# balcilar/gnn-matlang

Hardware: AMD Instinct MI355X
Metric: GNNML3 training graphs/sec on ZINC-12k (higher is better)
Workload: dtype f32 storage/accumulate; forward products fp32-class (edge branch bf16x6, conv f16x3 split), backward products bf16x3 split; 1 GPU; Zinc12k.py GNNML3 regression train step (4x ML3Layer 30+2, S=8 supports, learnedge, add-pool, L1-sum, Adam 1e-3), ZINC-like synthetic graphs; graphs_per_gpu=131072, global_batch=131072, nodes_per_gpu=3005312, support_edges_per_gpu=18320896, supports=8, parallelism=dp1, params=33309

## Files before the change

### gnn_matlang_amd/csrc/gml_spectconv_bwd3_impl.h

```cpp
#pragma once
#include <type_traits>
#include "gml_common.h"
#include "gml_spectconv_bwd_impl.h"

__host__ __device__ __forceinline__ int gml_wkey3(int o) { return ((o >> 3) & 1) << 1; }
__host__ __device__ __forceinline__ int gml_tkey3(int pos) { return ((pos >> 2) & 1) | ((((pos >> 1) ^ (pos >> 2) ^ (pos >> 3)) & 1) << 1); }

template <int S, int NFB, int NW, int NOB = 2>
struct GmlBwd3Cfg {
    static constexpr int ROWS = 16 * NW, NT = 64 * NW;
    static constexpr int ECAP_MAX = (S > 8 ? 12 : (S == 6 ? 16 : 8)) * ROWS;
    static constexpr int XCAP_MAX = 224;
    static constexpr int LDG = 16 * NOB + 4;
    static constexpr int NIMG = NFB > 2 ? 2 : 1;
    static constexpr int W_IMG = S * 16 * NOB * 32;
    static constexpr int W_HALF = NIMG * W_IMG;
    static constexpr int W_BYTES = 2 * W_HALF * 2;
    static constexpr int SS = (S % 4 == 0) ? 4 : ((S % 3 == 0) ? 3 : S);
    static constexpr int NSLAB = S / SS;
    static constexpr int NBLK = SS * NFB * NOB;
    static constexpr int BPW = (NBLK + NW - 1) / NW;
    static constexpr int XT_IMG = 2 * ROWS * 64;
    static constexpr int XT_BYTES = NIMG * XT_IMG;
    static constexpr int PT_BYTES = 2 * SS * ROWS * 64;
    static constexpr int GREC = 4 + ROWS / 4;
    static constexpr bool ASHARE = NW % (NOB * NFB) == 0;
    static constexpr bool OK = (S % SS == 0) && (NFB >= 1 && NFB <= 3) && NW == 8 && (NOB == 1 || NOB == 2) &&
                               (NFB < 3 || (NOB == 2 && S <= 6));
    __host__ __device__ static size_t stage_bytes(int ecap, int xcap) { return (size_t)ecap * S * 4 + (size_t)xcap * LDG * 4; }
    __host__ __device__ static size_t r_bytes(int ecap, int xcap) {
        const size_t a = stage_bytes(ecap, xcap);
        return a > (size_t)PT_BYTES ? a : (size_t)PT_BYTES;
    }
    static constexpr bool VALG = NOB == 2 && NW == 8 && (S == 8 || ((S == 6 || S == 4) && NFB == 3));
    __host__ __device__ static size_t lds_bytes(int ecap, int xcap) {
        if (VALG) return (size_t)W_BYTES + (ROWS + 8) * 4 + (size_t)ecap * 4 + (size_t)xcap * LDG * 4 + XT_BYTES + PT_BYTES;
        return (size_t)W_BYTES + (ROWS + 8) * 4 + (size_t)ecap * 4 + r_bytes(ecap, xcap) + XT_BYTES;
    }
};

#ifndef GML_ABL
#define GML_ABL 0
#endif

#ifdef GML_BWD2_TIMING
#define GML_T3(i) do { const unsigned t_ = (unsigned)__builtin_readcyclecounter(); tacc_[i] += t_ - tprev_; tprev_ = t_; } while (0)
#else
#define GML_T3(i)
#endif

#define GML_DPP9_(ctrl)                                                                                                          \
    asm("s_nop 1\n\tv_add_f32_dpp %0, %0, %0 " ctrl " row_mask:0xf bank_mask:0xf\n\tv_add_f32_dpp %1, %1, %1 " ctrl " row_mask:0xf bank_mask:0xf\n\t" \
        "v_add_f32_dpp %2, %2, %2 " ctrl " row_mask:0xf bank_mask:0xf\n\tv_add_f32_dpp %3, %3, %3 " ctrl " row_mask:0xf bank_mask:0xf\n\t"           \
        "v_add_f32_dpp %4, %4, %4 " ctrl " row_mask:0xf bank_mask:0xf\n\tv_add_f32_dpp %5, %5, %5 " ctrl " row_mask:0xf bank_mask:0xf\n\t"           \
        "v_add_f32_dpp %6, %6, %6 " ctrl " row_mask:0xf bank_mask:0xf\n\tv_add_f32_dpp %7, %7, %7 " ctrl " row_mask:0xf bank_mask:0xf\n\t"           \
        "v_add_f32_dpp %8, %8, %8 " ctrl " row_mask:0xf bank_mask:0xf"                                                         \
        : "+v"(v[0]), "+v"(v[1]), "+v"(v[2]), "+v"(v[3]), "+v"(v[4]), "+v"(v[5]), "+v"(v[6]), "+v"(v[7]), "+v"(v[8]))
__device__ __forceinline__ void gml_row16_sum9(float (&v)[9]) {
    GML_DPP9_("quad_perm:[1,0,3,2]");
    GML_DPP9_("quad_perm:[2,3,0,1]");
    GML_DPP9_("row_half_mirror");
    GML_DPP9_("row_mirror");
}

#ifndef GML_HADV
#define GML_HADV 0
#endif
#define GML_BWD3_HAD_LDS(ROWS_, NW_) (16 + (ROWS_) * 16 + (NW_) * 36 * 4)

template <int S, int NFB, int NW, bool XV, bool DZ = false, int NOB = 2, bool HAD = false>
__global__ __launch_bounds__(64 * NW, 2) void gml_k_spectconv_bwd3(const GmlBwdParams p) {
    static_assert(!HAD || (XV && NOB == 2 && NFB == 2 && S >= 2), "the fused output stage is compiled for the ZINC shape class");
    using C = GmlBwd3Cfg<S, NFB, NW, NOB>;
    constexpr int NH = 2 * NOB, GC = 4 * NOB;
    static_assert(!DZ || NOB == 2, "the dz hand-over is compiled for the ZINC shape class");
    constexpr int LDG = C::LDG, ROWS = C::ROWS, NT = C::NT, SS = C::SS, BPW = C::BPW;
    constexpr int VAL_ALIGN = (S % 4 == 0) ? 4 : ((S % 2 == 0) ? 2 : 1);
    constexpr bool VALG = C::VALG;
    constexpr bool DIRECT = NOB == 2 && (S == 8 || VALG);
    constexpr bool LATEC = VALG && C::NSLAB == 2;
    constexpr bool BUFLD = S == 8 && NOB == 2 && XV;
    extern __shared__ __attribute__((aligned(16))) unsigned char lds_raw[];
    __bf16* W_h = reinterpret_cast<__bf16*>(lds_raw);
    __bf16* W_l = W_h + C::W_HALF;
    int* rp_l = reinterpret_cast<int*>(lds_raw + C::W_BYTES);
    int* col_l = rp_l + ROWS + 8;
    unsigned char* rreg = reinterpret_cast<unsigned char*>(col_l + p.ecap);
    float* ea_l = reinterpret_cast<float*>(rreg);
    float* gs = VALG ? ea_l : ea_l + (size_t)p.ecap * S;
    unsigned char* xT = VALG ? rreg + (size_t)p.xcap * LDG * 4 : rreg + C::r_bytes(p.ecap, p.xcap);
    unsigned char* pT = VALG ? xT + C::XT_BYTES : rreg;
    float* wm_l = reinterpret_cast<float*>(VALG ? pT + C::PT_BYTES : xT + C::XT_BYTES);
    float* hb_l = wm_l + 128;
    float* dzf = hb_l + 4;
    float* bsum = dzf + ROWS * 4;

    const int tid = threadIdx.x;
    const int lane = tid & 63, wave = tid >> 6;
    const int r16 = lane & 15, kq = lane >> 4;
    const int wg = gml_xcd_remap(blockIdx.x, gridDim.x);
    const int g0 = wg * p.groups_per_wg;
    const int g1 = min(g0 + p.groups_per_wg, p.ngroups);

    if constexpr (DZ || HAD) {
        if (tid < 128) wm_l[tid] = ((tid >> 5) < p.nmix && (tid & 31) < p.Fin) ? ((tid >> 5) < p.nmix1 ? p.wmix[(tid >> 5) * p.Fin + (tid & 31)] : p.wmix2[((tid >> 5) - p.nmix1) * p.Fin + (tid & 31)]) : 0.f;
    }
    if constexpr (HAD) {
        if (tid < 4) hb_l[tid] = tid < 2 ? (p.hb11 ? p.hb11[tid] : 0.f) : (p.hb12 ? p.hb12[tid - 2] : 0.f);
        if (tid < NW * 36) bsum[tid] = 0.f;
    }
    constexpr int WO = 16 * NOB;
    constexpr int NIMG = C::NIMG;
    for (int e = tid; e < NIMG * S * WO * 32; e += NT) {
        const int fl = e & 31, o = (e >> 5) % WO, s = ((e >> 5) / WO) % S, img = (e >> 5) / (WO * S);
        const int f = 32 * img + fl;
        const float v = (f < p.Fin && o < p.Fout) ? p.w[((int64_t)s * p.Fin + f) * p.Fout + o] : 0.f;
        const __bf16 h = (__bf16)v;
        const __bf16 l = (__bf16)(v - (float)h);
        const int i = img * C::W_IMG + (s * WO + o) * 32 + ((((fl >> 3) ^ gml_wkey3(o)) & 3) << 3) + (fl & 7);
        W_h[i] = h; W_l[i] = l;
    }

    f32x4 dwacc[C::NSLAB][BPW];
#pragma unroll
    for (int i = 0; i < C::NSLAB; ++i)
#pragma unroll
        for (int j = 0; j < BPW; ++j) dwacc[i][j] = f32x4{0.f, 0.f, 0.f, 0.f};

#ifdef GML_BWD2_TIMING
    unsigned tacc_[12] = {0, 0, 0, 0, 0, 0, 0, 0, 0, 0, 0, 0};
    unsigned tprev_ = (unsigned)__builtin_readcyclecounter();
#endif
    constexpr int VW = (S % 4 == 0) ? 4 : ((S % 2 == 0) ? 2 : 1);
    typedef typename std::conditional<VW == 4, f32x4, f32x2>::type EV;
    constexpr int NC = C::ECAP_MAX / NT, NE4 = (VW > 1) ? C::ECAP_MAX * (S / VW) / NT : 1;
    constexpr int NG4 = (C::XCAP_MAX * GC + NT - 1) / NT;
    const int etot = p.rowptr[p.nrows];
    const int* colb = etot > 0 ? p.col : p.ginfo;
    const EV* valb = etot > 0 ? reinterpret_cast<const EV*>(p.val) : reinterpret_cast<const EV*>(p.ginfo);
    const int emax = max(etot, 1) - 1;
    const int64_t emax4 = (VW > 1) ? max((int64_t)etot * (S / VW), (int64_t)1) - 1 : 0;
    const int o4max = p.gvec ? ((p.Fout + 3) / 4 * 4 - 4) : 0;
    int cv[NC], rpv = 0, row_n = 0;
    EV ev4[NE4];
    f32x4 gv4[NG4];
    float xb[8];
    float xb2[NIMG == 2 ? 8 : 1];
    float gown[HAD ? 8 : 1];
    auto vec_group = [&](const int4 gi) {
        return (VW > 1) && p.gvec && gi.y <= C::ECAP_MAX && gi.w <= C::XCAP_MAX;
    };
    int4 gi_nv = int4{0, 0, 0, 0};
    int4 gi_c = int4{0, 0, 0, 0};
    auto latch = [&]() {
        gi_c = int4{__builtin_amdgcn_readfirstlane(gi_nv.x), __builtin_amdgcn_readfirstlane(gi_nv.y),
                    __builtin_amdgcn_readfirstlane(gi_nv.z), __builtin_amdgcn_readfirstlane(gi_nv.w)};
    };
    const int voff_g = (tid / GC) * (int)p.ldg * 4 + (tid % GC) * 16;
    auto issue = [&](int g) {
        const int64_t r0 = (int64_t)g * ROWS;
        const int4 gi = gi_c;
        const int kb = gi.x, ne = gi.y, lo = gi.z, nwin = gi.w;
        if constexpr (BUFLD) {
            auto rsrc = [](const void* base, int64_t nbytes) {
                return __builtin_amdgcn_make_buffer_rsrc(const_cast<void*>(base), 0, (int)(nbytes < 0 ? 0 : (nbytes > 0x7fffff00 ? 0x7fffff00 : nbytes)), 0x00020000);
            };
            const int64_t rem = (int64_t)etot - kb;
            const auto rs_rp = rsrc(p.rowptr + r0, (p.nrows + 1 - r0) * 4);
            const auto rs_col = rsrc(p.col + kb, rem * 4);
            const auto rs_val = rsrc(p.val + (int64_t)kb * S, rem * (S * 4));
            const auto rs_g = rsrc(p.g + (int64_t)lo * p.ldg, (p.nrows - lo) * p.ldg * 4);
            const auto rs_x = rsrc(p.x + r0 * p.ldx, (p.nrows - r0) * p.ldx * 4);
            const int ldxb = (int)p.ldx * 4, ldgb = (int)p.ldg * 4;
#pragma unroll
            for (int q4 = 0; q4 < 2; ++q4) {
                const u32x4 t = __builtin_amdgcn_raw_buffer_load_b128(rs_x, row_n * ldxb + 32 * kq + 16 * q4, 0, 0);
                xb[4 * q4] = __uint_as_float(t.x); xb[4 * q4 + 1] = __uint_as_float(t.y);
                xb[4 * q4 + 2] = __uint_as_float(t.z); xb[4 * q4 + 3] = __uint_as_float(t.w);
            }
            if constexpr (HAD && !(GML_HADV & 2)) {
                const auto rs_go = rsrc(p.g + r0 * p.ldg, (p.nrows - r0) * p.ldg * 4);
#pragma unroll
                for (int q4 = 0; q4 < 2; ++q4) {
                    const u32x4 t = __builtin_amdgcn_raw_buffer_load_b128(rs_go, row_n * ldgb + 32 * kq + 16 * q4, 0, 0);
                    gown[4 * q4] = __uint_as_float(t.x); gown[4 * q4 + 1] = __uint_as_float(t.y);
                    gown[4 * q4 + 2] = __uint_as_float(t.z); gown[4 * q4 + 3] = __uint_as_float(t.w);
                }
            }
            rpv = (int)__builtin_amdgcn_raw_buffer_load_b32(rs_rp, tid * 4, 0, 0);
#pragma unroll
            for (int t = 0; t < NC; ++t) cv[t] = (int)__builtin_amdgcn_raw_buffer_load_b32(rs_col, tid * 4, NT * 4 * t, 0);
#pragma unroll
            for (int t = 0; t < (VALG ? 0 : NE4); ++t) ev4[t] = __builtin_bit_cast(EV, __builtin_amdgcn_raw_buffer_load_b128(rs_val, tid * 16, NT * 16 * t, 0));
#pragma unroll
            for (int t = 0; t < NG4; ++t) gv4[t] = __builtin_bit_cast(f32x4, __builtin_amdgcn_raw_buffer_load_b128(rs_g, voff_g, t * (NT / GC) * ldgb, 0));
            return;
        }
        if constexpr (XV) {
            const float* xr = p.x + min(r0 + row_n, p.nrows - 1) * p.ldx;
            const int f4max = (p.Fin + 3) / 4 * 4 - 4;
#pragma unroll
            for (int q4 = 0; q4 < 2; ++q4) {
                const f32x4 t = *reinterpret_cast<const f32x4*>(xr + min(8 * kq + 4 * q4, f4max));
                xb[4 * q4] = t.x; xb[4 * q4 + 1] = t.y; xb[4 * q4 + 2] = t.z; xb[4 * q4 + 3] = t.w;
                if constexpr (NIMG == 2) {
                    const f32x4 u = *reinterpret_cast<const f32x4*>(xr + min(32 + 8 * kq + 4 * q4, f4max));
                    xb2[4 * q4] = u.x; xb2[4 * q4 + 1] = u.y; xb2[4 * q4 + 2] = u.z; xb2[4 * q4 + 3] = u.w;
                }
            }
        }
        if constexpr (HAD && !(GML_HADV & 2)) {
            const float* gr = p.g + min(r0 + row_n, p.nrows - 1) * p.ldg + 8 * kq;
#pragma unroll
            for (int q4 = 0; q4 < 2; ++q4) {
                const f32x4 t = *reinterpret_cast<const f32x4*>(gr + 4 * q4);
                gown[4 * q4] = t.x; gown[4 * q4 + 1] = t.y; gown[4 * q4 + 2] = t.z; gown[4 * q4 + 3] = t.w;
            }
        }
        rpv = p.rowptr[min(r0 + tid, p.nrows)];
        const int ne1 = max(ne, 1) - 1, ne41 = max(ne * (S / (VW > 1 ? VW : 1)), 1) - 1, nw1 = max(nwin, 1) - 1;
#pragma unroll
        for (int t = 0; t < NC; ++t) cv[t] = colb[min(kb + min(tid + NT * t, ne1), emax)];
#pragma unroll
        for (int t = 0; t < (VALG ? 0 : NE4); ++t) ev4[t] = valb[min((int64_t)kb * (S / (VW > 1 ? VW : 1)) + min(tid + NT * t, ne41), emax4)];
#pragma unroll
        for (int t = 0; t < NG4; ++t) {
            const int i = tid + NT * t;
            const int64_t rr = min((int64_t)lo + min(i / GC, nw1), p.nrows - 1);
            gv4[t] = *reinterpret_cast<const f32x4*>(p.g + rr * p.ldg + min((i % GC) * 4, o4max));
        }
    };
    auto load_rows = [&](int g) {
        const int32_t* rec = p.ginfo + (int64_t)g * C::GREC;
        gi_nv = *reinterpret_cast<const int4*>(rec);
        row_n = reinterpret_cast<const unsigned char*>(rec + 4)[wave * 16 + r16];
    };
    auto commit = [&](const int4 gi, const int nr) {
        const int kb = gi.x, ne = gi.y, lo = gi.z, nwin = gi.w;
        if (tid <= nr) rp_l[tid] = rpv;
        if (vec_group(gi)) {
#pragma unroll
            for (int t = 0; t < NC; ++t) { const int i = tid + NT * t; if (i < ne) col_l[i] = cv[t] - lo; }
#pragma unroll
            for (int t = 0; t < (VALG ? 0 : NE4); ++t) {
                const int i = tid + NT * t;
                if (i < ne * (S / (VW > 1 ? VW : 1))) reinterpret_cast<EV*>(ea_l)[i] = ev4[t];
            }
#pragma unroll
            for (int t = 0; t < NG4; ++t) {
                const int i = tid + NT * t;
                if (i < nwin * GC)
                    *reinterpret_cast<f32x4*>(gs + (i / GC) * LDG + (i % GC) * 4) = ((i % GC) * 4 < p.Fout) ? gv4[t] : f32x4{0.f, 0.f, 0.f, 0.f};
            }
        } else {
            for (int i = tid; i < ne; i += NT) col_l[i] = p.col[kb + i] - lo;
            if constexpr (!VALG)
                for (int i = tid; i < ne * S; i += NT) ea_l[i] = p.val[(int64_t)kb * S + i];
            for (int i = tid; i < nwin * 16 * NOB; i += NT) {
                const int rr = i / (16 * NOB), o = i % (16 * NOB);
                gs[rr * LDG + o] = (o < p.Fout) ? p.g[(int64_t)(lo + rr) * p.ldg + o] : 0.f;
            }
        }
    };
    if (g0 < g1) { load_rows(g0); latch(); issue(g0); }
    if constexpr (LATEC) {
        if (g0 < g1) commit(gi_c, (int)min((int64_t)ROWS, p.nrows - (int64_t)g0 * ROWS));
        __syncthreads();
    }
    if constexpr (HAD && !LATEC) __syncthreads();
    for (int g = g0; g < g1; ++g) {
        const int64_t r0 = (int64_t)g * ROWS;
        const int nr = (int)min((int64_t)ROWS, p.nrows - r0);
        const int4 gi = gi_c;
        const int kb = gi.x, ne = gi.y, lo = gi.z, nwin = gi.w;
        const int row = row_n;
        load_rows((GML_ABL & 1) ? g0 : min(g + 1, g1 - 1));
        const auto vrs = __builtin_amdgcn_make_buffer_rsrc(const_cast<float*>(VALG ? p.val + (int64_t)kb * S : p.x), 0, VALG ? ne * (S * 4) : 0, 0x00020000);
        uint32_t vtouch = 0;
        if constexpr (VALG) vtouch = __builtin_amdgcn_raw_buffer_load_b32(vrs, tid * 128, 0, 0);
        if constexpr (!VALG) __syncthreads();
        GML_T3(0);

        const bool rvalid = row < nr;
        if constexpr (!XV) {
            const float* xr = p.x + (r0 + row) * p.ldx + 8 * kq;
#pragma unroll
            for (int t = 0; t < 8; ++t) xb[t] = (rvalid && 8 * kq + t < p.Fin) ? xr[t] : 0.f;
            if constexpr (NIMG == 2) {
#pragma unroll
                for (int t = 0; t < 8; ++t) xb2[t] = (rvalid && 32 + 8 * kq + t < p.Fin) ? xr[32 + t] : 0.f;
            }
        }
        f32x4 dzv = f32x4{0.f, 0.f, 0.f, 0.f};
        float had_a[4], had_g6 = 0.f, had_g7 = 0.f, had_bs[9];
        const int pos_h = wave * 16 + r16;
        auto had_pre = [&]() {
#pragma unroll
            for (int j = 0; j < 8; ++j) {
                if (!(rvalid && 8 * kq + j < p.Fin)) xb[j] = 0.f;
                if ((!BUFLD && !rvalid) || (GML_HADV & 2)) gown[j] = 0.f;
            }
#pragma unroll
            for (int q = 0; q < 4; ++q) {
                const f32x4 w0 = *reinterpret_cast<const f32x4*>(wm_l + q * 32 + 8 * kq);
                const f32x4 w1 = *reinterpret_cast<const f32x4*>(wm_l + q * 32 + 8 * kq + 4);
                f32x2 a2 = f32x2{xb[0], xb[1]} * f32x2{w0.x, w0.y};
                a2 = f32x2{xb[2], xb[3]} * f32x2{w0.z, w0.w} + a2;
                a2 = f32x2{xb[4], xb[5]} * f32x2{w1.x, w1.y} + a2;
                a2 = f32x2{xb[6], xb[7]} * f32x2{w1.z, w1.w} + a2;
                had_a[q] = a2.x + a2.y;
            }
            had_g6 = __shfl(gown[6], r16 + 48); had_g7 = __shfl(gown[7], r16 + 48);
        };
        auto had_valu = [&]() {
            const auto a01 = __builtin_amdgcn_permlane16_swap(__float_as_uint(had_a[0]), __float_as_uint(had_a[1]), false, false);
            const auto a23 = __builtin_amdgcn_permlane16_swap(__float_as_uint(had_a[2]), __float_as_uint(had_a[3]), false, false);
            const float c01 = __uint_as_float(a01[0]) + __uint_as_float(a01[1]);
            const float c23 = __uint_as_float(a23[0]) + __uint_as_float(a23[1]);
            const auto bq = __builtin_amdgcn_permlane32_swap(__float_as_uint(c01), __float_as_uint(c23), false, false);
            const float pre = __uint_as_float(bq[0]) + __uint_as_float(bq[1]) + hb_l[kq];
            float th, dh;
            gml_tanh_d(pre, th, dh);
            const auto tsw = __builtin_amdgcn_permlane32_swap(__float_as_uint(th), __float_as_uint(th), false, false);
            const float tpart = __uint_as_float(kq < 2 ? tsw[1] : tsw[0]);
            const float dzo = (GML_HADV & 4) ? 0.f : ((kq & 1) ? had_g7 : had_g6) * tpart * dh;
            dzf[pos_h * 4 + kq] = dzo;
            if constexpr (!(GML_HADV & 1)) {
#pragma unroll
                for (int j = 0; j < 8; ++j) had_bs[j] = gown[j];
                had_bs[8] = dzo;
                gml_row16_sum9(had_bs);
            }
        };
        auto had_post = [&]() {
            if constexpr (!(GML_HADV & 1)) {
                if (r16 == 0) {
                    float* bw = bsum + wave * 36;
                    f32x4 o0 = *reinterpret_cast<const f32x4*>(bw + 8 * kq), o1 = *reinterpret_cast<const f32x4*>(bw + 8 * kq + 4);
                    o0 += f32x4{had_bs[0], had_bs[1], had_bs[2], had_bs[3]};
                    o1 += f32x4{had_bs[4], had_bs[5], had_bs[6], had_bs[7]};
                    *reinterpret_cast<f32x4*>(bw + 8 * kq) = o0;
                    *reinterpret_cast<f32x4*>(bw + 8 * kq + 4) = o1;
                    bw[32 + kq] += had_bs[8];
                }
            }
            dzv = *reinterpret_cast<const f32x4*>(dzf + pos_h * 4);
        };
        if constexpr (!LATEC) commit(gi, nr);
        bf16x8 xh, xl;
        bf16x8 xh2, xl2;
        unsigned xpos = 0;
        f32x2 Z[S][NH], P[S][NH];
        auto zproj = [&]() {
        if constexpr (HAD) had_pre();
        if constexpr (XV) {
#pragma unroll
            for (int j = 0; j < 8; ++j)
                if (!(rvalid && 8 * kq + j < p.Fin)) xb[j] = 0.f;
        }
        gml_split8(xb, xh, xl);
        if constexpr (NIMG == 2) {
#pragma unroll
            for (int j = 0; j < 8; ++j)
                if (!(rvalid && 32 + 8 * kq + j < p.Fin)) xb2[j] = 0.f;
            gml_split8(xb2, xh2, xl2);
        }
        if constexpr (DZ) {
#pragma unroll
            for (int j = 0; j < 8; ++j) xpos |= (xb[j] > 0.f ? 1u : 0u) << j;
        }

        {
            const int oa0 = NOB == 2 ? 8 * (r16 >> 2) + (r16 & 3) : r16;
            bf16x8 wh[2][NOB], wl[2][NOB];
            bf16x8 wh2[2][NIMG == 2 ? NOB : 1], wl2[2][NIMG == 2 ? NOB : 1];
            auto frag = [&](int s, int st) {
#pragma unroll
                for (int ob = 0; ob < NOB; ++ob) {
                    const int oa = oa0 + 4 * ob;
                    const int off = (s * WO + oa) * 32 + (((kq ^ gml_wkey3(oa)) & 3) << 3);
                    wh[st][ob] = *reinterpret_cast<const bf16x8*>(W_h + off);
                    wl[st][ob] = *reinterpret_cast<const bf16x8*>(W_l + off);
                    if constexpr (NIMG == 2) {
                        wh2[st][ob] = *reinterpret_cast<const bf16x8*>(W_h + C::W_IMG + off);
                        wl2[st][ob] = *reinterpret_cast<const bf16x8*>(W_l + C::W_IMG + off);
                    }
                }
            };
            if (!(GML_ABL & 16)) frag(0, 0);
            if constexpr (HAD) had_valu();
#pragma unroll
            for (int s = 0; s < S; ++s) {
                const int st = s & 1;
                if (GML_ABL & 16) {
#pragma unroll
                    for (int h = 0; h < NH; ++h) { Z[s][h] = f32x2{xb[h], xb[h + 4]}; P[s][h] = f32x2{0.f, 0.f}; }
                    continue;
                }
                if (s + 1 < S) frag(s + 1, st ^ 1);
                f32x4 dd[NOB];
#pragma unroll
                for (int ob = 0; ob < NOB; ++ob) dd[ob] = f32x4{0.f, 0.f, 0.f, 0.f};
#pragma unroll
                for (int ob = 0; ob < NOB; ++ob) dd[ob] = __builtin_amdgcn_mfma_f32_16x16x32_bf16(wl[st][ob], xh, dd[ob], 0, 0, 0);
#pragma unroll
                for (int ob = 0; ob < NOB; ++ob) dd[ob] = __builtin_amdgcn_mfma_f32_16x16x32_bf16(wh[st][ob], xl, dd[ob], 0, 0, 0);
#pragma unroll
                for (int ob = 0; ob < NOB; ++ob) dd[ob] = __builtin_amdgcn_mfma_f32_16x16x32_bf16(wh[st][ob], xh, dd[ob], 0, 0, 0);
                if constexpr (NIMG == 2) {
#pragma unroll
                    for (int ob = 0; ob < NOB; ++ob) dd[ob] = __builtin_amdgcn_mfma_f32_16x16x32_bf16(wl2[st][ob], xh2, dd[ob], 0, 0, 0);
#pragma unroll
                    for (int ob = 0; ob < NOB; ++ob) dd[ob] = __builtin_amdgcn_mfma_f32_16x16x32_bf16(wh2[st][ob], xl2, dd[ob], 0, 0, 0);
#pragma unroll
                    for (int ob = 0; ob < NOB; ++ob) dd[ob] = __builtin_amdgcn_mfma_f32_16x16x32_bf16(wh2[st][ob], xh2, dd[ob], 0, 0, 0);
                }
#pragma unroll
                for (int ob = 0; ob < NOB; ++ob) { Z[s][2 * ob] = f32x2{dd[ob][0], dd[ob][1]}; Z[s][2 * ob + 1] = f32x2{dd[ob][2], dd[ob][3]}; }
#pragma unroll
                for (int h = 0; h < NH; ++h) asm volatile("v_pk_mov_b32 %0, 0, 0" : "=v"(P[s][h]));
            }
            __builtin_amdgcn_sched_group_barrier(0x100, 2 * NOB * NIMG, 0);
#pragma unroll
            for (int s = 0; s < S; ++s) {
                if (s + 1 < S) __builtin_amdgcn_sched_group_barrier(0x100, 2 * NOB * NIMG, 0);
                __builtin_amdgcn_sched_group_barrier(0x008, 3 * NOB * NIMG, 0);
            }
        }
        if constexpr (HAD) had_post();
        };
        if constexpr (!LATEC) __syncthreads();
        GML_T3(1);
        f32x4 dxa[NFB];
        const bool dxv = p.dx && p.dxvec;
        if constexpr (DZ) {
            if constexpr (!HAD) dzv = *reinterpret_cast<const f32x4*>(p.dz + min(r0 + row, p.nrows - 1) * 4);
        } else if constexpr (!HAD) {
            const float* dxb = p.dx ? p.dx : p.x;
            const int64_t ldb = p.dx ? p.lddx : p.ldx;
            const float* dr = dxb + min(r0 + row, p.nrows - 1) * ldb;
            if (dxv) {
                const int f4max = (p.Fin + 3) / 4 * 4 - 4;
#pragma unroll
                for (int fb = 0; fb < NFB; ++fb) dxa[fb] = *reinterpret_cast<const f32x4*>(dr + min(16 * fb + 4 * kq, f4max));
            } else {
#pragma unroll
                for (int fb = 0; fb < NFB; ++fb)
#pragma unroll
                    for (int reg = 0; reg < 4; ++reg) dxa[fb][reg] = dr[min(16 * fb + 4 * kq + reg, p.Fin - 1)];
            }
        }

        const int kbeg = rvalid ? rp_l[row] - kb : 0;
        const int kend = rvalid ? rp_l[row + 1] - kb : 0;

        zproj();
        GML_T3(2);
        const auto dvrs = __builtin_amdgcn_make_buffer_rsrc(const_cast<float*>(DIRECT && p.dval ? p.dval + (int64_t)kb * S : p.x), 0,
                                                            (DIRECT && p.dval && !(GML_ABL & 8)) ? ne * (S * 4) : 0, 0x00020000);
        auto ldg_row = [&](int dstl, f32x2 (&gv)[NH]) {
#pragma unroll
            for (int ob = 0; ob < NOB; ++ob) {
                const f32x4 t0 = *reinterpret_cast<const f32x4*>(gs + dstl * LDG + 4 * NOB * kq + 4 * ob);
                gv[2 * ob] = f32x2{t0.x, t0.y}; gv[2 * ob + 1] = f32x2{t0.z, t0.w};
            }
        };
        auto edge_g = [&](int k, const float (&ev)[S], const f32x2 (&gv)[NH]) {
            float d[S];
#pragma unroll
            for (int s = 0; s < S; ++s) {
                f32x2 a2 = f32x2{0.f, 0.f};
                const f32x2 e2 = f32x2{ev[s], ev[s]};
#pragma unroll
                for (int h = 0; h < NH; ++h) {
                    P[s][h] = e2 * gv[h] + P[s][h];
                    a2 = Z[s][h] * gv[h] + a2;
                }
                d[s] = a2.x + a2.y;
            }
            if constexpr (DIRECT && S == 4) {
                const auto a01 = __builtin_amdgcn_permlane16_swap(__float_as_uint(d[0]), __float_as_uint(d[1]), false, false);
                const auto a23 = __builtin_amdgcn_permlane16_swap(__float_as_uint(d[2]), __float_as_uint(d[3]), false, false);
                const float c01 = __uint_as_float(a01[0]) + __uint_as_float(a01[1]);
                const float c23 = __uint_as_float(a23[0]) + __uint_as_float(a23[1]);
                const auto b = __builtin_amdgcn_permlane32_swap(__float_as_uint(c01), __float_as_uint(c23), false, false);
                __builtin_amdgcn_raw_buffer_store_b32(__float_as_uint(__uint_as_float(b[0]) + __uint_as_float(b[1])), dvrs, (k * S + kq) * 4, 0, 0);
            } else if constexpr (DIRECT) {
                float tot2[2];
#pragma unroll
                for (int c = 0; c < 2; ++c) {
                    const float d6 = (S > 6) ? d[(S > 6) ? 6 + c : 0] : 0.f;
                    const auto a01 = __builtin_amdgcn_permlane16_swap(__float_as_uint(d[c]), __float_as_uint(d[2 + c]), false, false);
                    const auto a23 = __builtin_amdgcn_permlane16_swap(__float_as_uint(d[4 + c]), __float_as_uint(d6), false, false);
                    const float c01 = __uint_as_float(a01[0]) + __uint_as_float(a01[1]);
                    const float c23 = __uint_as_float(a23[0]) + __uint_as_float(a23[1]);
                    const auto b = __builtin_amdgcn_permlane32_swap(__float_as_uint(c01), __float_as_uint(c23), false, false);
                    tot2[c] = __uint_as_float(b[0]) + __uint_as_float(b[1]);
                }
                typedef uint32_t u32x2_ __attribute__((ext_vector_type(2)));
                const int doff = (S == 8 || kq < S / 2) ? (k * S + 2 * kq) * 4 : 0x7ffffff0;
                __builtin_amdgcn_raw_buffer_store_b64(u32x2_{__float_as_uint(tot2[0]), __float_as_uint(tot2[1])}, dvrs, doff, 0, 0);
            } else {
#pragma unroll
            for (int c = 0; c < (S + 3) / 4; ++c) {
                const float v0 = d[4 * c], v1 = (4 * c + 1 < S) ? d[4 * c + 1] : 0.f;
                const float v2 = (4 * c + 2 < S) ? d[4 * c + 2] : 0.f, v3 = (4 * c + 3 < S) ? d[4 * c + 3] : 0.f;
                const auto a01 = __builtin_amdgcn_permlane16_swap(__float_as_uint(v0), __float_as_uint(v1), false, false);
                const auto a23 = __builtin_amdgcn_permlane16_swap(__float_as_uint(v2), __float_as_uint(v3), false, false);
                const float c01 = __uint_as_float(a01[0]) + __uint_as_float(a01[1]);
                const float c23 = __uint_as_float(a23[0]) + __uint_as_float(a23[1]);
                const auto b = __builtin_amdgcn_permlane32_swap(__float_as_uint(c01), __float_as_uint(c23), false, false);
                const float tot = __uint_as_float(b[0]) + __uint_as_float(b[1]);
                if (4 * c + kq < S) ea_l[k * S + 4 * c + kq] = tot;
            }
            }
        };
        auto edge = [&](int k, const float (&ev)[S]) {
            f32x2 gv[NH];
            ldg_row(col_l[k], gv);
            edge_g(k, ev, gv);
        };
        if constexpr (VALG) {
            asm volatile("" :: "v"(vtouch));
            auto ldval = [&](int k, float (&ev)[S]) {
                const u32x4 a = __builtin_amdgcn_raw_buffer_load_b128(vrs, k * (S * 4), 0, 0);
                ev[0] = __uint_as_float(a.x); ev[1] = __uint_as_float(a.y); ev[2] = __uint_as_float(a.z); ev[3] = __uint_as_float(a.w);
                if constexpr (S == 8) {
                    const u32x4 b = __builtin_amdgcn_raw_buffer_load_b128(vrs, k * (S * 4) + 16, 0, 0);
                    ev[4] = __uint_as_float(b.x); ev[5] = __uint_as_float(b.y); ev[6] = __uint_as_float(b.z); ev[7] = __uint_as_float(b.w);
                } else if constexpr (S == 6) {
                    typedef uint32_t u32x2v __attribute__((ext_vector_type(2)));
                    const u32x2v b = __builtin_amdgcn_raw_buffer_load_b64(vrs, k * (S * 4) + 16, 0, 0);
                    ev[4] = __uint_as_float(b.x); ev[5] = __uint_as_float(b.y);
                }
            };
            int k = kbeg;
            const int klast = kend - 1;
            if (k < ((GML_ABL & 4) ? kbeg : kend)) {
                float eA[S], eB[S];
                ldval(k, eA);
                for (;;) {
                    ldval(min(k + 1, klast), eB);
                    edge(k, eA);
                    if (++k >= kend) break;
                    ldval(min(k + 1, klast), eA);
                    edge(k, eB);
                    if (++k >= kend) break;
                }
            }
        } else {
            for (int k = kbeg; k < ((GML_ABL & 4) ? kbeg : kend); ++k) {
                float ev[S];
                gml_load_row<S, VAL_ALIGN>(ea_l + k * S, ev);
                edge(k, ev);
            }
        }
        GML_T3(3);
        __syncthreads();
        GML_T3(4);
        int tid_o = tid;
        asm volatile("" : "+v"(tid_o));
        const int r16o = tid_o & 15, kqo = (tid_o >> 4) & 3, waveo = __builtin_amdgcn_readfirstlane(tid_o >> 6);
        typedef typename std::conditional<NOB == 2, bf16x8, bf16x4>::type PFrag;
        if constexpr (HAD) {
            if (kqo == 3) {
                P[0][3] = f32x2{dzv[0], dzv[1]};
                P[1][3] = f32x2{dzv[2], dzv[3]};
            }
        }
        PFrag PH[S], PL[S];
#pragma unroll
        for (int s = 0; s < S; ++s) {
            float pv[8];
#pragma unroll
            for (int h = 0; h < 4; ++h) {
                const f32x2 t = h < NH ? P[s][h < NH ? h : 0] : f32x2{0.f, 0.f};
                pv[2 * h] = t.x; pv[2 * h + 1] = t.y;
            }
            bf16x8 th, tl;
            gml_split8(pv, th, tl);
            if constexpr (NOB == 2) { PH[s] = th; PL[s] = tl; }
            else { PH[s] = bf16x4{th[0], th[1], th[2], th[3]}; PL[s] = bf16x4{tl[0], tl[1], tl[2], tl[3]}; }
        }
        GML_T3(10);
        const int pos = waveo * 16 + r16o;
        const int woff = pos * 64 + (((kqo ^ gml_tkey3(pos)) & 3) << 4);
        auto write_x = [&]() {
            *reinterpret_cast<bf16x8*>(xT + woff) = xh;
            *reinterpret_cast<bf16x8*>(xT + ROWS * 64 + woff) = xl;
            if constexpr (NIMG == 2) {
                *reinterpret_cast<bf16x8*>(xT + C::XT_IMG + woff) = xh2;
                *reinterpret_cast<bf16x8*>(xT + C::XT_IMG + ROWS * 64 + woff) = xl2;
            }
        };
        auto write_slab = [&](int sl) {
#pragma unroll
            for (int se = 0; se < SS; ++se) {
                const int s = sl * SS + se;
                if constexpr (NOB == 2) {
                    *reinterpret_cast<bf16x8*>(pT + se * ROWS * 64 + woff) = PH[s];
                    *reinterpret_cast<bf16x8*>(pT + (SS + se) * ROWS * 64 + woff) = PL[s];
                } else {
                    const int woff1 = pos * 64 + ((((kqo >> 1) ^ gml_tkey3(pos)) & 3) << 4) + ((kqo & 1) << 3);
                    *reinterpret_cast<bf16x4*>(pT + se * ROWS * 64 + woff1) = PH[s];
                    *reinterpret_cast<bf16x4*>(pT + (SS + se) * ROWS * 64 + woff1) = PL[s];
                }
            }
        };
        if constexpr (DIRECT) {
            if (p.dw_partial && !(GML_ABL & 2)) { write_x(); write_slab(0); }
        }
        latch();
        issue((GML_ABL & 1) ? g0 : min(g + 1, g1 - 1));
        GML_T3(8);

        if (!DIRECT && p.dval && !(GML_ABL & 8)) {
            constexpr bool ACC = !(S == 8 && NOB == 2);
            if (ACC && (p.flags & GML_DVAL_ACCUM)) {
                for (int i = tid_o; i < ne * S; i += NT) p.dval[(int64_t)kb * S + i] += ea_l[i];
            } else if constexpr (VW > 1) {
                EV* dst = reinterpret_cast<EV*>(p.dval + (int64_t)kb * S);
                for (int i = tid_o; i < ne * (S / VW); i += NT) dst[i] = reinterpret_cast<const EV*>(ea_l)[i];
            } else {
                for (int i = tid_o; i < ne * S; i += NT) p.dval[(int64_t)kb * S + i] = ea_l[i];
            }
        }

        GML_T3(9);
        if ((DZ || !HAD) && p.dx && !(GML_ABL & 32)) {
            if constexpr (DZ) {
#pragma unroll
                for (int fb = 0; fb < NFB; ++fb) {
                    f32x4 a = f32x4{0.f, 0.f, 0.f, 0.f};
#pragma unroll
                    for (int q = 0; q < 4; ++q) a += dzv[q] * *reinterpret_cast<const f32x4*>(wm_l + q * 32 + 16 * fb + 4 * kqo);
                    dxa[fb] = a;
                }
            } else if (!(p.flags & GML_ACCUM)) {
#pragma unroll
                for (int fb = 0; fb < NFB; ++fb) dxa[fb] = f32x4{0.f, 0.f, 0.f, 0.f};
            }
            const int tj = r16o >> 2, tc = r16o & 3;
            int aoff[2][NFB];
#pragma unroll
            for (int h = 0; h < 2; ++h)
#pragma unroll
                for (int fb = 0; fb < NFB; ++fb) {
                    const int o = NOB == 2 ? 8 * kqo + 4 * h + tj : 4 * kqo + tj, cidx = 4 * (fb & 1) + tc;
                    aoff[h][fb] = (fb >> 1) * (C::W_IMG * 2) + o * 64 + ((((cidx >> 1) ^ gml_wkey3(o)) & 3) << 4) + ((cidx & 1) << 3);
                }
            const unsigned char* Wh8 = reinterpret_cast<const unsigned char*>(W_h);
            const unsigned char* Wl8 = reinterpret_cast<const unsigned char*>(W_l);
            bf16x8 vh[2][NFB], vl[2][NFB];
            auto fragx = [&](int s, int st) {
#pragma unroll
                for (int fb = 0; fb < NFB; ++fb) {
                    vh[st][fb] = gml_tr_frag(Wh8 + s * (WO * 64) + aoff[0][fb], Wh8 + s * (WO * 64) + aoff[1][fb]);
                    vl[st][fb] = gml_tr_frag(Wl8 + s * (WO * 64) + aoff[0][fb], Wl8 + s * (WO * 64) + aoff[1][fb]);
                }
            };
            fragx(0, 0);
#pragma unroll
            for (int s = 0; s < S; ++s) {
                const int st = s & 1;
                if (s + 1 < S) fragx(s + 1, st ^ 1);
                bf16x8 ph, pl;
                if constexpr (NOB == 2) { ph = PH[s]; pl = PL[s]; }
                else {
                    const __bf16 z = (__bf16)0.f;
                    ph = bf16x8{PH[s][0], PH[s][1], PH[s][2], PH[s][3], z, z, z, z};
                    pl = bf16x8{PL[s][0], PL[s][1], PL[s][2], PL[s][3], z, z, z, z};
                }
#pragma unroll
                for (int fb = 0; fb < NFB; ++fb) dxa[fb] = __builtin_amdgcn_mfma_f32_16x16x32_bf16(vl[st][fb], ph, dxa[fb], 0, 0, 0);
#pragma unroll
                for (int fb = 0; fb < NFB; ++fb) dxa[fb] = __builtin_amdgcn_mfma_f32_16x16x32_bf16(vh[st][fb], pl, dxa[fb], 0, 0, 0);
#pragma unroll
                for (int fb = 0; fb < NFB; ++fb) dxa[fb] = __builtin_amdgcn_mfma_f32_16x16x32_bf16(vh[st][fb], ph, dxa[fb], 0, 0, 0);
            }
            __builtin_amdgcn_sched_group_barrier(0x100, 4 * NFB, 1);
#pragma unroll
            for (int s = 0; s < S; ++s) {
                if (s + 1 < S) __builtin_amdgcn_sched_group_barrier(0x100, 4 * NFB, 1);
                __builtin_amdgcn_sched_group_barrier(0x008, 3 * NFB, 1);
            }
            if constexpr (DZ) {
                if (p.relu_cols > 0) {
#pragma unroll
                    for (int fb = 0; fb < NFB; ++fb) {
                        const unsigned mm = (unsigned)__shfl((int)xpos, r16o + 16 * (2 * fb + (kqo >> 1))) >> (4 * (kqo & 1));
#pragma unroll
                        for (int reg = 0; reg < 4; ++reg)
                            if (16 * fb + 4 * kqo + reg < p.relu_cols && !((mm >> reg) & 1u)) dxa[fb][reg] = 0.f;
                    }
                }
            }
            float* dr = p.dx + (r0 + row) * p.lddx + 4 * kqo;
            if (GML_ABL & 8) {
#pragma unroll
                for (int fb = 0; fb < NFB; ++fb) asm volatile("" :: "v"(dxa[fb]));
            } else if (dxv) {
#pragma unroll
                for (int fb = 0; fb < NFB; ++fb)
                    if (rvalid && 16 * fb + 4 * kqo < p.Fin) *reinterpret_cast<f32x4*>(dr + 16 * fb) = dxa[fb];
            } else {
#pragma unroll
                for (int fb = 0; fb < NFB; ++fb)
#pragma unroll
                    for (int reg = 0; reg < 4; ++reg)
                        if (rvalid && 16 * fb + 4 * kqo + reg < p.Fin) dr[16 * fb + reg] = dxa[fb][reg];
            }
        }

        GML_T3(5);
        if (p.dw_partial && !(GML_ABL & 2)) {
            if constexpr (!DIRECT) write_x();
            const int tj = r16o >> 2, tc = r16o & 3;
            auto roffs = [&](int h, int blk) {
                const int ps = 8 * kqo + 4 * h + tj, cidx = 4 * blk + tc;
                return ps * 64 + ((((cidx >> 1) ^ gml_tkey3(ps)) & 3) << 4) + ((cidx & 1) << 3);
            };
            constexpr int NB_ = (C::NBLK >= NW) ? BPW : 1;
            constexpr int NA_ = C::ASHARE ? 1 : NB_;
            const int ob = wave % NOB;
            const int offB[2] = {roffs(0, ob), roffs(1, ob)};
            int offA[NA_][2], seo[NB_];
#pragma unroll
            for (int i = 0; i < NB_; ++i) {
                const int b = min(wave + NW * i, C::NBLK - 1);
                seo[i] = ((b / NOB) / NFB) * ROWS * 64;
                if (i < NA_) {
                    const int fb = (b / NOB) % NFB;
                    offA[i][0] = (fb >> 1) * C::XT_IMG + roffs(0, fb & 1);
                    offA[i][1] = (fb >> 1) * C::XT_IMG + roffs(1, fb & 1);
                }
            }
#pragma unroll
            for (int sl = 0; sl < C::NSLAB; ++sl) {
                if (!(DIRECT && sl == 0)) {
                    __syncthreads();
                    write_slab(sl);
                }
                if constexpr (LATEC) {
                    if (sl == C::NSLAB - 1) commit(gi_c, (int)min((int64_t)ROWS, p.nrows - (int64_t)min(g + 1, g1 - 1) * ROWS));
                }
                __syncthreads();
                GML_T3(11);
                if (wave < C::NBLK) {
                    bf16x8 fah[2][NA_], fal[2][NA_], fbh[2][NB_], fbl[2][NB_];
                    auto fragw = [&](int st, int sg) {
                        const unsigned char* xa = xT + st * 2048;
#pragma unroll
                        for (int i = 0; i < NA_; ++i) {
                            fah[sg][i] = gml_tr_frag(xa + offA[i][0], xa + offA[i][1]);
                            fal[sg][i] = gml_tr_frag(xa + ROWS * 64 + offA[i][0], xa + ROWS * 64 + offA[i][1]);
                        }
#pragma unroll
                        for (int i = 0; i < NB_; ++i) {
                            const unsigned char* pa = pT + seo[i] + st * 2048;
                            fbh[sg][i] = gml_tr_frag(pa + offB[0], pa + offB[1]);
                            fbl[sg][i] = gml_tr_frag(pa + SS * ROWS * 64 + offB[0], pa + SS * ROWS * 64 + offB[1]);
                        }
                    };
                    f32x4 d[NB_];
#pragma unroll
                    for (int i = 0; i < NB_; ++i) d[i] = dwacc[sl][i];
                    fragw(0, 0);
#pragma unroll
                    for (int st = 0; st < ROWS / 32; ++st) {
                        const int sg = st & 1;
                        if (st + 1 < ROWS / 32) fragw(st + 1, sg ^ 1);
#pragma unroll
                        for (int i = 0; i < NB_; ++i) d[i] = __builtin_amdgcn_mfma_f32_16x16x32_bf16(fal[sg][i < NA_ ? i : 0], fbh[sg][i], d[i], 0, 0, 0);
#pragma unroll
                        for (int i = 0; i < NB_; ++i) d[i] = __builtin_amdgcn_mfma_f32_16x16x32_bf16(fah[sg][i < NA_ ? i : 0], fbl[sg][i], d[i], 0, 0, 0);
#pragma unroll
                        for (int i = 0; i < NB_; ++i) d[i] = __builtin_amdgcn_mfma_f32_16x16x32_bf16(fah[sg][i < NA_ ? i : 0], fbh[sg][i], d[i], 0, 0, 0);
                    }
                    __builtin_amdgcn_sched_group_barrier(0x100, 4 * NA_ + 4 * NB_, 2);
#pragma unroll
                    for (int st = 0; st < ROWS / 32; ++st) {
                        if (st + 1 < ROWS / 32) __builtin_amdgcn_sched_group_barrier(0x100, 4 * NA_ + 4 * NB_, 2);
                        __builtin_amdgcn_sched_group_barrier(0x008, 3 * NB_, 2);
                    }
#pragma unroll
                    for (int i = 0; i < NB_; ++i)
                        if (wave + NW * i < C::NBLK) dwacc[sl][i] = d[i];
                }
                GML_T3(7);
            }
        } else if constexpr (LATEC) {
            commit(gi_c, (int)min((int64_t)ROWS, p.nrows - (int64_t)min(g + 1, g1 - 1) * ROWS));
            __syncthreads();
        }
    }

    GML_T3(6);
#ifdef GML_BWD2_TIMING
    if (lane == 0) {
#pragma unroll
        for (int i = 0; i < 12; ++i) atomicAdd(&p.prof[i], (unsigned long long)tacc_[i]);
    }
#endif
    if (p.dw_partial && g0 < g1) {
        float* out = p.dw_partial + (int64_t)wg * S * p.Fin * p.Fout;
#pragma unroll
        for (int sl = 0; sl < C::NSLAB; ++sl)
#pragma unroll
            for (int i = 0; i < BPW; ++i) {
                const int b = wave + NW * i;
                if (b < C::NBLK) {
                    const int ob = b % NOB, fb = (b / NOB) % NFB, s = sl * SS + (b / NOB) / NFB;
                    const int o = ob * 16 + r16;
#pragma unroll
                    for (int reg = 0; reg < 4; ++reg) {
                        const int f = fb * 16 + 4 * kq + reg;
                        if (f < p.Fin && o < p.Fout) out[((int64_t)s * p.Fin + f) * p.Fout + o] = dwacc[sl][i][reg];
                        if constexpr (HAD) {
                            if (f < p.Fin && o >= 30 && s < 2)
                                p.hpart[(int64_t)wg * (4 * p.Fin + 4 + p.Fout) + (2 * s + (o - 30)) * p.Fin + f] = dwacc[sl][i][reg];
                        }
                    }
                }
            }
    }
    if constexpr (HAD) {
        __syncthreads();
        if (g0 < g1 && tid < 36) {
            float v = 0.f;
#pragma unroll
            for (int w = 0; w < NW; ++w) v += bsum[w * 36 + tid];
            float* hp = p.hpart + (int64_t)wg * (4 * p.Fin + 4 + p.Fout) + 4 * p.Fin;
            if (tid >= 32) hp[tid - 32] = v;
            else if (tid < p.Fout) hp[4 + tid] = v;
        }
    }
}

template <int S, int NFB, int NW, int NOB = 2>
int gml_launch_bwd3(const GmlBwdParams& p, dim3 grid, size_t lds, hipStream_t st);

template <int S, int NFB, int NW, bool EN>
struct GmlBwd3Dz {
    static int go(const GmlBwdParams&, dim3, size_t, hipStream_t) { return GML_E_UNSUPPORTED; }
};
template <int S, int NFB, int NW>
struct GmlBwd3Dz<S, NFB, NW, true> {
    static int go(const GmlBwdParams& p, dim3 grid, size_t lds, hipStream_t st) {
        if (!p.xvec || !p.dxvec || p.nmix < 1 || p.nmix > 4 || !p.wmix || !p.dx) return GML_E_UNSUPPORTED;
        GML_ALLOW_BIG_LDS(rc, (&gml_k_spectconv_bwd3<S, NFB, NW, true, true>), 160 * 1024)
        if (rc != hipSuccess) return (int)rc;
        hipLaunchKernelGGL((gml_k_spectconv_bwd3<S, NFB, NW, true, true>), grid, dim3(64 * NW), lds, st, p);
        return gml_launch_status();
    }
};
#define GML_BWD3_HAS_DZ(SV, NFBV, NWV) ((SV) == 8 && (NFBV) == 2 && (NWV) == 8)

int gml_launch_bwd3_had(const GmlBwdParams& p, dim3 grid, size_t lds, hipStream_t st);

#define GML_DEFINE_BWD3(SV, NFBV, NWV)                                                                       \
    template <>                                                                                              \
    int gml_launch_bwd3<SV, NFBV, NWV>(const GmlBwdParams& p, dim3 grid, size_t lds, hipStream_t st) {       \
        static_assert(GmlBwd3Cfg<SV, NFBV, NWV>::OK, "unsupported shape");                                   \
        if (p.dz != nullptr) return GmlBwd3Dz<SV, NFBV, NWV, GML_BWD3_HAS_DZ(SV, NFBV, NWV)>::go(p, grid, lds, st);  \
        GML_ALLOW_BIG_LDS(rc1, (&gml_k_spectconv_bwd3<SV, NFBV, NWV, true>), 160 * 1024)                     \
        GML_ALLOW_BIG_LDS(rc0, (&gml_k_spectconv_bwd3<SV, NFBV, NWV, false>), 160 * 1024)                    \
        if (rc1 != hipSuccess) return (int)rc1;                                                              \
        if (rc0 != hipSuccess) return (int)rc0;                                                              \
        if (p.xvec) hipLaunchKernelGGL((gml_k_spectconv_bwd3<SV, NFBV, NWV, true>), grid, dim3(64 * NWV), lds, st, p);  \
        else hipLaunchKernelGGL((gml_k_spectconv_bwd3<SV, NFBV, NWV, false>), grid, dim3(64 * NWV), lds, st, p);        \
        return gml_launch_status();                                                                          \
    }

#define GML_DEFINE_BWD3_N1(SV, NFBV, NWV)                                                                    \
    template <>                                                                                              \
    int gml_launch_bwd3<SV, NFBV, NWV, 1>(const GmlBwdParams& p, dim3 grid, size_t lds, hipStream_t st) {    \
        static_assert(GmlBwd3Cfg<SV, NFBV, NWV, 1>::OK, "unsupported shape");                                \
        if (p.dz != nullptr) return GML_E_UNSUPPORTED;                                                       \
        GML_ALLOW_BIG_LDS(rc1, (&gml_k_spectconv_bwd3<SV, NFBV, NWV, true, false, 1>), 160 * 1024)           \
        GML_ALLOW_BIG_LDS(rc0, (&gml_k_spectconv_bwd3<SV, NFBV, NWV, false, false, 1>), 160 * 1024)          \
        if (rc1 != hipSuccess) return (int)rc1;                                                              \
        if (rc0 != hipSuccess) return (int)rc0;                                                              \
        if (p.xvec) hipLaunchKernelGGL((gml_k_spectconv_bwd3<SV, NFBV, NWV, true, false, 1>), grid, dim3(64 * NWV), lds, st, p);  \
        else hipLaunchKernelGGL((gml_k_spectconv_bwd3<SV, NFBV, NWV, false, false, 1>), grid, dim3(64 * NWV), lds, st, p);        \
        return gml_launch_status();                                                                          \
    }
```

Baseline: 15.03 million graphs/s.

## Land next group's gradient window and column indices in LDS via async DMA

For the S=8 ZINC backward spectral-conv path, the register-staged prefetch of rowptr, col and gradient rows (later committed to LDS) is replaced with direct global-to-LDS DMA loads issued right after the next group's issue step. The transfer is meant to overlap the current group's MFMA weight-gradient work and to drop the register round-trip and commit copy. Edge gathers then read gradient rows from the padded LDS window by computed byte offset. Non-vectorisable groups fall back to a scalar copy. This adds an LDS zero-fill at kernel start and a vmcnt(0) wait before the last slab, which may stall if the DMA has not finished.

```diff
diff --git a/gnn_matlang_amd/csrc/gml_spectconv_bwd3_impl.h b/gnn_matlang_amd/csrc/gml_spectconv_bwd3_impl.h
--- a/gnn_matlang_amd/csrc/gml_spectconv_bwd3_impl.h
+++ b/gnn_matlang_amd/csrc/gml_spectconv_bwd3_impl.h
@@ -2,6 +2,7 @@
 #include <type_traits>
 #include "gml_common.h"
 #include "gml_spectconv_bwd_impl.h"
+#include "gml_spectconv_fwd3_impl.h"
 
 __host__ __device__ __forceinline__ int gml_wkey3(int o) { return ((o >> 3) & 1) << 1; }
 __host__ __device__ __forceinline__ int gml_tkey3(int pos) { return ((pos >> 2) & 1) | ((((pos >> 1) ^ (pos >> 2) ^ (pos >> 3)) & 1) << 1); }
@@ -33,6 +34,9 @@
         return a > (size_t)PT_BYTES ? a : (size_t)PT_BYTES;
     }
     static constexpr bool VALG = NOB == 2 && NW == 8 && (S == 8 || ((S == 6 || S == 4) && NFB == 3));
+    static constexpr bool LANDC = VALG && S == 8 && NSLAB == 2;
+    static constexpr int COL_AT = ROWS + 4;
+    static_assert(!LANDC || LDG == 36, "seven padded window rows per landing instruction");
     __host__ __device__ static size_t lds_bytes(int ecap, int xcap) {
         if (VALG) return (size_t)W_BYTES + (ROWS + 8) * 4 + (size_t)ecap * 4 + (size_t)xcap * LDG * 4 + XT_BYTES + PT_BYTES;
         return (size_t)W_BYTES + (ROWS + 8) * 4 + (size_t)ecap * 4 + r_bytes(ecap, xcap) + XT_BYTES;
@@ -80,6 +84,7 @@
     constexpr bool DIRECT = NOB == 2 && (S == 8 || VALG);
     constexpr bool LATEC = VALG && C::NSLAB == 2;
     constexpr bool BUFLD = S == 8 && NOB == 2 && XV;
+    constexpr bool LAND = BUFLD && C::LANDC && LATEC;
     extern __shared__ __attribute__((aligned(16))) unsigned char lds_raw[];
     __bf16* W_h = reinterpret_cast<__bf16*>(lds_raw);
     __bf16* W_l = W_h + C::W_HALF;
@@ -119,6 +124,11 @@
         const __bf16 l = (__bf16)(v - (float)h);
         const int i = img * C::W_IMG + (s * WO + o) * 32 + ((((fl >> 3) ^ gml_wkey3(o)) & 3) << 3) + (fl & 7);
         W_h[i] = h; W_l[i] = l;
+    }
+    if constexpr (LAND) {
+        const int n16 = p.xcap * LDG / 4;
+        for (int i = tid; i < n16; i += NT) reinterpret_cast<f32x4*>(gs)[i] = f32x4{0.f, 0.f, 0.f, 0.f};
+        __syncthreads();
     }
 
     f32x4 dwacc[C::NSLAB][BPW];
@@ -187,13 +197,15 @@
                     gown[4 * q4 + 2] = __uint_as_float(t.z); gown[4 * q4 + 3] = __uint_as_float(t.w);
                 }
             }
-            rpv = (int)__builtin_amdgcn_raw_buffer_load_b32(rs_rp, tid * 4, 0, 0);
-#pragma unroll
-            for (int t = 0; t < NC; ++t) cv[t] = (int)__builtin_amdgcn_raw_buffer_load_b32(rs_col, tid * 4, NT * 4 * t, 0);
-#pragma unroll
-            for (int t = 0; t < (VALG ? 0 : NE4); ++t) ev4[t] = __builtin_bit_cast(EV, __builtin_amdgcn_raw_buffer_load_b128(rs_val, tid * 16, NT * 16 * t, 0));
-#pragma unroll
-            for (int t = 0; t < NG4; ++t) gv4[t] = __builtin_bit_cast(f32x4, __builtin_amdgcn_raw_buffer_load_b128(rs_g, voff_g, t * (NT / GC) * ldgb, 0));
+            if constexpr (!LAND) {
+                rpv = (int)__builtin_amdgcn_raw_buffer_load_b32(rs_rp, tid * 4, 0, 0);
+#pragma unroll
+                for (int t = 0; t < NC; ++t) cv[t] = (int)__builtin_amdgcn_raw_buffer_load_b32(rs_col, tid * 4, NT * 4 * t, 0);
+#pragma unroll
+                for (int t = 0; t < (VALG ? 0 : NE4); ++t) ev4[t] = __builtin_bit_cast(EV, __builtin_amdgcn_raw_buffer_load_b128(rs_val, tid * 16, NT * 16 * t, 0));
+#pragma unroll
+                for (int t = 0; t < NG4; ++t) gv4[t] = __builtin_bit_cast(f32x4, __builtin_amdgcn_raw_buffer_load_b128(rs_g, voff_g, t * (NT / GC) * ldgb, 0));
+            }
             return;
         }
         if constexpr (XV) {
@@ -262,8 +274,59 @@
             }
         }
     };
-    if (g0 < g1) { load_rows(g0); latch(); issue(g0); }
-    if constexpr (LATEC) {
+    const int wave_s = __builtin_amdgcn_readfirstlane(tid >> 6);
+    int* const colw_l = rp_l + C::COL_AT;
+    auto land = [&](int g) {
+        if constexpr (LAND) {
+            const uint32_t lds0 = (uint32_t)(uintptr_t)((gml_lds_void*)lds_raw);
+            auto nb = [](int64_t nbytes) { return (uint32_t)(nbytes < 0 ? 0 : (nbytes > 0x7fffff00 ? 0x7fffff00 : nbytes)); };
+            const int64_t r0 = (int64_t)g * ROWS;
+            const int kb = gi_c.x, ne = gi_c.y, lo = gi_c.z, nwin = gi_c.w;
+            const bool vg = vec_group(gi_c) && ne > 0 && nwin > 0;
+            const int kb4 = kb & ~3, ne4 = vg ? ne + (kb & 3) : 0;
+            const int nwv = vg ? nwin : 0;
+            const int nxi = (nwv + 6) / 7, nci = (ne4 + 255) >> 8;
+            const u32x4 rs_g = gml_raw_rsrc(p.g + (int64_t)lo * p.ldg, nb((p.nrows - lo) * p.ldg * 4));
+            const u32x4 rs_col = gml_raw_rsrc(p.col + kb4, nb(((int64_t)etot - kb4) * 4));
+            const u32x4 rs_rp = gml_raw_rsrc(p.rowptr + r0, nb((p.nrows + 1 - r0) * 4));
+            const int ldgb = (int)p.ldg * 4;
+            const int wj = (lane * 57) >> 9, wch = lane - 9 * wj;
+            const int voff_w = wj * ldgb + wch * 16;
+            const bool won = wj < 7 && wch < 8 && wch * 4 < p.Fout;
+            const uint32_t col0 = lds0 + (uint32_t)(reinterpret_cast<unsigned char*>(colw_l) - lds_raw);
+            const uint32_t gs0 = lds0 + (uint32_t)(reinterpret_cast<unsigned char*>(gs) - lds_raw);
+            for (int t = wave_s; t < nxi + nci + 1; t += NW) {
+                if (t < nxi) {
+                    if (won && 7 * t + wj < nwv) gml_dma16(rs_g, gs0 + t * (7 * LDG * 4), voff_w + 7 * t * ldgb);
+                } else if (t < nxi + nci) {
+                    const int j = t - nxi;
+                    if (256 * j + 4 * lane < ne4) gml_dma16(rs_col, col0 + j * 1024, (256 * j + 4 * lane) * 4);
+                } else {
+                    if (lane < ROWS / 4 + 1) gml_dma16(rs_rp, lds0 + C::W_BYTES, lane * 16);
+                }
+            }
+            asm volatile("" ::: "memory");
+        }
+    };
+    auto land_wait = [&](const int4 gi) {
+        if constexpr (LAND) {
+            const int kb = gi.x, ne = gi.y, lo = gi.z, nwin = gi.w;
+            if (!vec_group(gi)) {
+                const int k3 = kb & 3;
+                for (int i = tid; i < ne; i += NT) colw_l[k3 + i] = p.col[kb + i];
+                for (int i = tid; i < nwin * 32; i += NT) {
+                    const int rr = i >> 5, o = i & 31;
+                    gs[rr * LDG + o] = (o < p.Fout) ? p.g[(int64_t)(lo + rr) * p.ldg + o] : 0.f;
+                }
+            }
+            asm volatile("s_waitcnt vmcnt(0)" ::: "memory");
+        }
+    };
+    if (g0 < g1) { load_rows(g0); latch(); issue(g0); land(g0); }
+    if constexpr (LAND) {
+        if (g0 < g1) land_wait(gi_c);
+        __syncthreads();
+    } else if constexpr (LATEC) {
         if (g0 < g1) commit(gi_c, (int)min((int64_t)ROWS, p.nrows - (int64_t)g0 * ROWS));
         __syncthreads();
     }
@@ -515,9 +578,21 @@
             }
             }
         };
+        const int* colk = LAND ? colw_l + (kb & 3) : col_l;
+        const uint32_t gwl = (uint32_t)(reinterpret_cast<const unsigned char*>(gs) - lds_raw) + 4 * NOB * 4 * kq - (uint32_t)lo * (LDG * 4);
         auto edge = [&](int k, const float (&ev)[S]) {
             f32x2 gv[NH];
-            ldg_row(col_l[k], gv);
+            if constexpr (LAND) {
+                const uint32_t c = (uint32_t)colk[k];
+                const unsigned char* gr = lds_raw + (uint32_t)(gwl + (c << 7) + (c << 4));
+#pragma unroll
+                for (int ob = 0; ob < NOB; ++ob) {
+                    const f32x4 t0 = *reinterpret_cast<const f32x4*>(gr + 16 * ob);
+                    gv[2 * ob] = f32x2{t0.x, t0.y}; gv[2 * ob + 1] = f32x2{t0.z, t0.w};
+                }
+            } else {
+                ldg_row(col_l[k], gv);
+            }
             edge_g(k, ev, gv);
         };
         if constexpr (VALG) {
@@ -612,6 +687,7 @@
         }
         latch();
         issue((GML_ABL & 1) ? g0 : min(g + 1, g1 - 1));
+        land((GML_ABL & 1) ? g0 : min(g + 1, g1 - 1));
         GML_T3(8);
 
         if (!DIRECT && p.dval && !(GML_ABL & 8)) {
@@ -741,7 +817,9 @@
                     __syncthreads();
                     write_slab(sl);
                 }
-                if constexpr (LATEC) {
+                if constexpr (LAND) {
+                    if (sl == C::NSLAB - 1) land_wait(gi_c);
+                } else if constexpr (LATEC) {
                     if (sl == C::NSLAB - 1) commit(gi_c, (int)min((int64_t)ROWS, p.nrows - (int64_t)min(g + 1, g1 - 1) * ROWS));
                 }
                 __syncthreads();
@@ -789,6 +867,9 @@
                 }
                 GML_T3(7);
             }
+        } else if constexpr (LAND) {
+            land_wait(gi_c);
+            __syncthreads();
         } else if constexpr (LATEC) {
             commit(gi_c, (int)min((int64_t)ROWS, p.nrows - (int64_t)min(g + 1, g1 - 1) * ROWS));
             __syncthreads();
```

After: 14.99 million graphs/s. No clear change (-0.3%).
